# 3DOM-FBK/deep-image-matching

Hardware: AMD Instinct MI355X
Metric: image-pairs/s (SuperPoint+LightGlue, 1024^2, 2048 kpts) (higher is better)
Workload: dtype f32

## Files before the change

### deep-image-matching_amd/csrc/api_ops.hip

```cpp
#include <stdarg.h>
#include <stdio.h>

#include "../../include/dim_hip.h"
#include "sp_kernels.h"

static thread_local char g_err[1024] = "";

void dim_set_error(const char* fmt, ...) {
  va_list ap;
  va_start(ap, fmt);
  vsnprintf(g_err, sizeof(g_err), fmt, ap);
  va_end(ap);
}

#include <vector>
namespace {
unsigned long long g_prof_mask = 0ull;
std::vector<hipEvent_t> g_prof_ev;
size_t g_prof_used = 0;
}

namespace {
constexpr int kMaxDev = 16;
unsigned* g_sat_dev[kMaxDev] = {nullptr};
// ... 85 lines not shown
int dim_follow_stop_flags() { return tuned(18, g_follow_stop); }
static int g_defer_assign = 1;
int dim_defer_assignment() { return tuned(17, g_defer_assign); }
static int g_fuse_ffn_ln = 3;
int dim_fuse_ffn_ln() { return tuned(11, g_fuse_ffn_ln); }
#ifdef DIM_RESEARCH
static int g_gemm_kc = 32;
int dim_gemm_kc() { return g_gemm_kc; }
static int g_conv_wino = 0;
int dim_conv_winograd() { return g_conv_wino; }
static int g_gemm_probe = 0;
int dim_gemm_probe() { return g_gemm_probe; }
static int g_attn_probe = 0;
int dim_attn_probe() { return g_attn_probe; }
#endif
static int g_al_tile_rows = 16;
int dim_aliked_tile_rows() { return tuned(10, g_al_tile_rows); }
static int g_al_fuse_bn = 1;
int dim_aliked_fuse_bn() { return tuned(9, g_al_fuse_bn); }
static int g_presplit = 1;
int dim_presplit_activations() { return tuned(5, g_presplit); }

void dim_prof_begin(int site, hipStream_t s) {
  if (!((g_prof_mask >> site) & 1ull)) return;
  if (g_prof_used + 2 > g_prof_ev.size()) {
    hipEvent_t a, b;
    if (hipEventCreate(&a) != hipSuccess || hipEventCreate(&b) != hipSuccess) return;
    g_prof_ev.push_back(a); g_prof_ev.push_back(b);
  }
  hipEventRecord(g_prof_ev[g_prof_used], s);
// ... 235 lines not shown
  if (key == 0) dim_conv_set_variant(value);
  if (key == 1) g_precision_mode = value;
  if (key == 2) dim_conv_x6_set_variant(value);
  if (key == 3) g_fuse_conv1a = value;
  if (key == 4) g_fold_out_proj = value;
  if (key == 5) g_presplit = value;
  if (key == 6) dim_gemm_x6_set_wide(value);
  if (key == 7) dim_nms_set_big_tiles(value);
  if (key == 8) g_fuse_kv = value;
  if (key == 9) g_al_fuse_bn = value;
  if (key == 10) g_al_tile_rows = value;
  if (key == 11) g_fuse_ffn_ln = value;
  if (key == 16) g_fuse_sp_head = value;
  if (key == 17) g_defer_assign = value;
  if (key == 18) g_follow_stop = value;
#ifdef DIM_RESEARCH
  if (key == 12) g_attn_probe = value;
  if (key == 13) g_gemm_probe = value;
  if (key == 14) g_gemm_kc = value;
  if (key == 15) g_conv_wino = value;
#else
  DIM_REQUIRE(key < 12 || key > 15, "dim_tune_set: key %d selects a research prototype / timing probe that the product library does not contain "
              "(build.build_variant(\"research\", [\"-DDIM_RESEARCH\"]) -> libdim_hip_research.so)", key);
#endif
  DIM_REQUIRE(key >= 0 && key <= 18, "dim_tune_set: unknown key %d", key);
  return 0;
}

int dim_handle_tune_set(void* handle, int key, int value) {
  DimHandleBase* b = (DimHandleBase*)handle;
  DIM_REQUIRE(b != nullptr && b->magic == DIM_HANDLE_MAGIC, "dim_handle_tune_set: not an extractor / matcher handle of this library");
  DIM_REQUIRE(key == 1 || key == 3 || key == 4 || key == 5 || key == 8 || key == 9 || key == 10 || key == 11 || key == 16 || key == 17 || key == 18,
              "dim_handle_tune_set: key %d has no per-handle form (arithmetic 1; fusion 3, 4, 5, 8, 9, 11, 16, 17, 18; ALIKED tile rows 10)", key);
  b->tune.v[key] = value < 0 ? -1 : value;
  return 0;
}

int dim_device_synchronize(void) {
  DIM_HIP(hipDeviceSynchronize());
  return 0;
}

}
```

### deep-image-matching_amd/csrc/conv_x6.hip

```cpp
#include <math.h>
#include <string.h>

#include <type_traits>

#include "dim_kernels.h"

namespace {
constexpr int TW = 32, IW = TW + 2;
constexpr int tile_rows(int mr) { return 4 * mr; }
__host__ __device__ constexpr size_t planes_image_pixels(int h, int w) { return ((size_t)h * w + 1) & ~(size_t)1; }
constexpr int w_slice(int npl) { return npl * 3 * 2 * 64 * 8; }

template <int CIN, int POOL, int PF, bool F1A, int MODE, bool PIN, bool POUT, int MR = 2, bool WDMA = false, bool BN = false>
__global__ __launch_bounds__(256, ((PF == 2 || MR == 4) ? 2 : 3)) void conv3x3_x6_kernel(const float* __restrict__ in, const unsigned short* __restrict__ wx,
                                                            const float* __restrict__ bias, float* __restrict__ out, int H, int W,
                                                            int cout, int relu, int tiles_x, const float* __restrict__ w1a,
                                                            const float* __restrict__ b1a, const float* __restrict__ inv_ch, unsigned* sat,
                                                            unsigned* sat_image) {
  static_assert(!(PIN || POUT) || MODE == 2, "pre-split planes exist for the fp16x3 mode only");
  static_assert(!(PIN && F1A), "the fused conv1a computes its own input");
  using S = SplitMma<MODE>;
  constexpr int NPL = S::NPL, W_SLICE = w_slice(NPL);
  constexpr int TH = tile_rows(MR), IH = TH + 2, NPIX = IH * IW;
  __shared__ u32x4 Ip[NPL * 2 * NPIX];
// ... 266 lines not shown
          const int y = oy + MR * wv + m;
#pragma unroll
          for (int r = 0; r < 16; r += 2) {
            const int x0 = ox + mfma_row(r, half);
            float v0 = acc[m][n][r] * inv_scale + bv, v1 = acc[m][n][r + 1] * inv_scale + bv;
            finish(v0, v1);
            put2((unsigned)(y * W + x0), x0, W, co, cpart, v0, v1);
          }
        }
      }
    }
    if (MODE == 2) sat_report(sat, vmax * (1.0f / OSC));
  };
  if (POOL ? ((ox >> 1) + TW / 2 <= Wo) : (ox + TW <= W)) run_epilogue(std::false_type{});
  else run_epilogue(std::true_type{});
}

__global__ __launch_bounds__(256) void planes_to_f32_kernel(const unsigned short* __restrict__ planes, int C, int hw, float* __restrict__ out, size_t n) {
  const size_t i = (size_t)blockIdx.x * 256 + threadIdx.x;
  if (i >= n) return;
  const size_t gp = i / C, c = i - gp * C, b = gp / hw, pix = gp - b * hw;
  const size_t o = b * planes_image_pixels(hw, 1) * 2 * C + (pix >> 1) * 4 * C + (c >> 4) * 64 + (pix & 1) * 32 + (c & 15);
  const _Float16 hv = __builtin_bit_cast(_Float16, planes[o]), lv = __builtin_bit_cast(_Float16, planes[o + 16]);
  out[i] = ((float)hv + (float)lv) / DIM_F16_ACT_SCALE;
}

unsigned short host_bf16_rne(float x) {
  unsigned u;
  memcpy(&u, &x, 4);
  if ((u & 0x7f800000u) == 0x7f800000u) return (unsigned short)(u >> 16);
// ... 135 lines not shown
    else if (planes_in && planes_out) DIM_CONV6P(CI, P, true, true); \
    else if (planes_in) DIM_CONV6P(CI, P, true, false);        \
    else if (planes_out) DIM_CONV6P(CI, P, false, true);       \
    else DIM_CONV6P(CI, P, false, false);                      \
  }
  if (cin == 64 && pool) DIM_CONV6P_IO(64, 1)
  else if (cin == 64) DIM_CONV6P_IO(64, 0)
  else if (pool) DIM_CONV6P_IO(128, 1)
  else DIM_CONV6P_IO(128, 0)
#undef DIM_CONV6P_IO
#undef DIM_CONV6P
  DIM_LAUNCH_CHECK();
  return 0;
}

int launch_planes_to_f32(const void* planes, int batch, int hw, int channels, float* out, hipStream_t s) {
  const size_t n = (size_t)batch * hw * channels;
  if (n == 0) return 0;
  hipLaunchKernelGGL(planes_to_f32_kernel, dim3((unsigned)((n + 255) / 256)), dim3(256), 0, s, (const unsigned short*)planes, channels, hw, out, n);
  DIM_LAUNCH_CHECK();
  return 0;
}
```

### deep-image-matching_amd/csrc/dim_common.h

```cpp
#pragma once
#include <hip/hip_runtime.h>
#include <stdint.h>

#include <memory>
#include <vector>

typedef float f32x16 __attribute__((ext_vector_type(16)));
typedef float f32x4 __attribute__((ext_vector_type(4)));

typedef __attribute__((ext_vector_type(8))) __bf16 bf16x8;
typedef unsigned int u32x4 __attribute__((ext_vector_type(4)));

#define DIM_WAVE 64

__device__ __forceinline__ f32x16 mfma32(float a, float b, f32x16 c) {
  return __builtin_amdgcn_mfma_f32_32x32x2f32(a, b, c, 0, 0, 0);
}
__device__ __forceinline__ f32x16 mfma_bf16(u32x4 a, u32x4 b, f32x16 c) {
  return __builtin_amdgcn_mfma_f32_32x32x16_bf16(__builtin_bit_cast(bf16x8, a), __builtin_bit_cast(bf16x8, b), c, 0, 0, 0);
}
typedef __attribute__((ext_vector_type(2))) __bf16 bf16x2;
typedef float f32x2 __attribute__((ext_vector_type(2)));
__device__ __forceinline__ unsigned cvt_pk_bf16(float a, float b) {
  f32x2 v = {a, b};
// ... 202 lines not shown
  do {                                                                                \
    hipError_t e__ = hipGetLastError();                                               \
    if (e__ != hipSuccess) {                                                          \
      dim_set_error("kernel launch failed: %s (%s:%d)", hipGetErrorString(e__), __FILE__, __LINE__); \
      return -1;                                                                      \
    }                                                                                 \
  } while (0)
#define DIM_REQUIRE(cond, ...)            \
  do {                                    \
    if (!(cond)) {                        \
      dim_set_error(__VA_ARGS__);         \
      return -2;                          \
    }                                     \
  } while (0)

constexpr int DIM_TUNE_KEYS = 19;
constexpr unsigned DIM_HANDLE_MAGIC = 0x44494d48u;
struct DimTune {
  int v[DIM_TUNE_KEYS];
  DimTune() { for (int i = 0; i < DIM_TUNE_KEYS; ++i) v[i] = -1; }
};
struct DimHandleBase {
  unsigned magic = DIM_HANDLE_MAGIC;
  DimTune tune;
  std::vector<void*> allocs;
  size_t bytes = 0;
};
constexpr size_t DIM_ALLOC_SLACK = 256;
int dim_dev_alloc_bytes(DimHandleBase* b, void** p, size_t bytes);
template <typename T> int dim_dev_alloc(DimHandleBase* b, T** p, size_t count) {
  void* q = nullptr;
// ... 33 lines not shown
```

### deep-image-matching_amd/csrc/dim_kernels.h

```cpp
#pragma once
#include "dim_common.h"

struct SplitWeights {
  const unsigned short* dev = nullptr;
  int mode = 0;
  size_t scale_off = 0;
  int n_pad = 0;
  const float* inv_ch() const { return (const float*)(dev + scale_off); }
};
struct GemmLayerTab { const unsigned short* Bx3; const float* inv_ch; const float* bias; };
struct GemmArgs {
  const float* A0 = nullptr; const float* A1 = nullptr;
  int lda0 = 0, lda1 = 0, ksplit = 0;
  long long strideA0 = 0, strideA1 = 0;
  const int* a_idx = nullptr;
  const float* B = nullptr; int ldb = 0; long long strideB = 0; int bt = 0;
  const unsigned short* Bx3 = nullptr; int n_pad = 0;
  int split_mode = 1; const float* inv_ch = nullptr;
  void set_split(const SplitWeights& w) { Bx3 = w.dev; n_pad = w.n_pad; split_mode = w.mode; inv_ch = w.inv_ch(); }
  unsigned* sat = nullptr;
  const float* bias = nullptr;
  const float* R = nullptr; int ldr = 0; long long strideR = 0;
  float* C = nullptr; int ldc = 0; long long strideC = 0;
  int M = 0, N = 0, K = 0;
// ... 15 lines not shown
int launch_gemm_x6_nt(const GemmArgs& a, int batch, int split_mode, hipStream_t s);
size_t gemm_split_weight_elems(int K, int n_pad, int mode);
void split_weights(const float* w_kn, int K, int N, int n_pad, int mode, unsigned short* out, SplitWeights* sw, int kperm = 0);

int launch_conv3x3(const float* in, const float* w, const float* bias, float* out, int batch, int H, int W,
                   int cin, int cout, int pool, int relu, hipStream_t s);
size_t conv_split_weight_elems(int cin, int cout, int mode);
void prepare_conv_weights_split(const float* w_oihw, int cin, int cout, int mode, unsigned short* out, SplitWeights* sw);
int launch_conv3x3_x6(const float* in, const SplitWeights& wt, const float* bias, float* out, int batch, int H, int W, int cin,
                      int cout, int pool, int relu, hipStream_t s, unsigned* sat = nullptr, int bn = 0);
int launch_conv3x3_x6_fused1a(const float* image, const float* w1a_tap_cout, const float* b1a, const SplitWeights& wt, const float* bias,
                              float* out, int batch, int H, int W, int cout, int pool, int relu, int planes_out, hipStream_t s,
                              unsigned* sat = nullptr, unsigned* sat_image = nullptr, int bn = 0);
int launch_conv3x3_x6_planes(const float* in, const SplitWeights& wt, const float* bias, float* out, int batch, int H, int W, int cin,
                             int cout, int pool, int relu, int planes_in, int planes_out, hipStream_t s, unsigned* sat = nullptr, int bn = 0);
size_t conv_wino_weight_elems(int cin, int cout);
void prepare_conv_weights_wino(const float* w_oihw, int cin, int cout, unsigned short* out, SplitWeights* sw);
int launch_conv3x3_wg_fused1a(const float* image, const float* w1a_tap_cout, const float* b1a, const SplitWeights& wt, const float* bias,
                              float* out, int batch, int H, int W, int cout, int pool, int planes_out, hipStream_t s, unsigned* sat = nullptr,
                              unsigned* sat_image = nullptr);
#ifdef DIM_RESEARCH
int dim_conv_winograd();
#else
static inline int dim_conv_winograd() { return 0; }
#endif
int launch_planes_to_f32(const void* planes, int batch, int hw, int channels, float* out, hipStream_t s);
inline size_t dim_planes_image_pixels(int h, int w) { return ((size_t)h * w + 1) & ~(size_t)1; }
int dim_presplit_activations();
int dim_precision_mode();
int dim_aliked_tile_rows();
// ... 29 lines not shown
```

### deep-image-matching_amd/csrc/sp_api.hip

```cpp
#include <math.h>
#include <stdlib.h>
#include <string.h>

#include <vector>

#include "../../include/dim_hip.h"
#include "sp_kernels.h"

struct dim_sp {
  DimHandleBase base;
  dim_sp_config cfg;
  int max_batch, max_h, max_w, capacity;
  float* w1a; float* wk[12]; float* bias[12];
  SplitWeights wsw[12];
  SplitWeights wsp[3][12];
  float *a1, *b1, *a2, *b2, *a3, *b3, *a4, *x, *pa, *logits, *da, *dd, *smap, *nms, *cand_score;
  int *cand_idx, *rowcount, *rowoff, *ncand;
  unsigned long long* topk_keys;
  int last_h, last_w, last_batch;
  float conv1a_bound;
  bool x_is_planes;
  bool head_fused;
  float* b1_dbg;
  float* x_dbg;
  bool bn;
};

namespace {
const int kCin[12] = {1, 64, 64, 64, 64, 128, 128, 128, 128, 256, 128, 256};
const int kCout[12] = {64, 64, 64, 64, 128, 128, 128, 128, 256, 65, 256, 256};
const int kK[12] = {3, 3, 3, 3, 3, 3, 3, 3, 3, 1, 3, 1};

int sp_create(const dim_sp_weights* w, const std::vector<float>* bn_st, const dim_sp_config* cfg, int max_batch, int max_h, int max_w, int capacity,
              dim_sp** out) {
  DIM_REQUIRE(w && cfg && out, "dim_sp_create: null argument");
  DIM_REQUIRE(max_batch > 0 && max_h >= 8 && max_w >= 8, "dim_sp_create: bad sizes");
  DIM_REQUIRE(cfg->max_keypoints != 0 && cfg->max_keypoints >= -1, "\"max_keypoints\" must be positive or \"-1\"");
  DIM_REQUIRE(capacity > 0 && capacity >= cfg->max_keypoints, "dim_sp_create: capacity %d < max_keypoints %d", capacity, cfg->max_keypoints);
  DIM_REQUIRE(cfg->nms_radius >= 0, "nms_radius must be >= 0");
  std::unique_ptr<dim_sp, void (*)(dim_sp*)> guard(new dim_sp(), dim_sp_destroy);
  dim_sp* const h = guard.get();
  DimHandleBase* const hb = &h->base;
  memset((void*)&h->cfg, 0, sizeof(h->cfg));
  h->cfg = *cfg;
  h->max_batch = max_batch; h->max_h = max_h; h->max_w = max_w; h->capacity = capacity;
  h->last_h = h->last_w = h->last_batch = 0;
  h->b1_dbg = nullptr; h->x_dbg = nullptr; h->head_fused = false;
  h->bn = bn_st != nullptr;
  for (int l = 0; l < 12; ++l) {
    const int ci = kCin[l], co = kCout[l], k = kK[l];
    const int co_pad = (co + 3) & ~3;
    if (!dim_all_finite(w->conv_w[l], (size_t)k * k * ci * co) || !dim_all_finite(w->conv_b[l], (size_t)co)) { dim_set_error("dim_sp_create: non-finite value in the weights of layer %d", l); return -1; }
    std::vector<float> host((size_t)k * k * ci * co_pad, 0.0f);
    for (int o = 0; o < co; ++o)
      for (int i = 0; i < ci; ++i)
        for (int t = 0; t < k * k; ++t) host[((size_t)t * ci + i) * co_pad + o] = w->conv_w[l][((size_t)o * ci + i) * k * k + t];
    if (k == 3 && ci >= 64) {
      for (int mode = 1; mode <= 2; ++mode) {
        std::vector<unsigned short> hx(conv_split_weight_elems(ci, co, mode));
        SplitWeights& sw = h->wsp[mode][l];
        prepare_conv_weights_split(w->conv_w[l], ci, co, mode, hx.data(), &sw);
        DIM_TRY(dim_upload_split(hb, &sw, hx, mode, sw.n_pad));
// ... 26 lines not shown
    if (bn_st) sum = fabsf(bn_st[0][o]) * sum + fabsf(bn_st[0][64 + o]);
    h->conv1a_bound = fmaxf(h->conv1a_bound, sum);
  }
  const size_t B = max_batch, H = max_h, W = max_w;
  const size_t H2 = H / 2, W2 = W / 2, H4 = H2 / 2, W4 = W2 / 2, hh = H4 / 2, ww = W4 / 2;
  h->a1 = nullptr;
  DIM_TRY(dim_dev_alloc(hb, &h->b1, B * dim_planes_image_pixels(H2, W2) * 64));
  DIM_TRY(dim_dev_alloc(hb, &h->a2, B * dim_planes_image_pixels(H2, W2) * 64));
  DIM_TRY(dim_dev_alloc(hb, &h->b2, B * dim_planes_image_pixels(H4, W4) * 64));
  DIM_TRY(dim_dev_alloc(hb, &h->a3, B * dim_planes_image_pixels(H4, W4) * 128));
  DIM_TRY(dim_dev_alloc(hb, &h->b3, B * dim_planes_image_pixels(hh, ww) * 128));
  DIM_TRY(dim_dev_alloc(hb, &h->a4, B * dim_planes_image_pixels(hh, ww) * 128));
  DIM_TRY(dim_dev_alloc(hb, &h->x, B * dim_planes_image_pixels(hh, ww) * 128));
  DIM_TRY(dim_dev_alloc(hb, &h->pa, B * hh * ww * 256));
  DIM_TRY(dim_dev_alloc(hb, &h->logits, B * hh * ww * 65));
  DIM_TRY(dim_dev_alloc(hb, &h->da, B * hh * ww * 256));
  DIM_TRY(dim_dev_alloc(hb, &h->dd, B * hh * ww * 256));
  DIM_TRY(dim_dev_alloc(hb, &h->smap, B * hh * ww * 64));
  DIM_TRY(dim_dev_alloc(hb, &h->nms, B * hh * ww * 64));
  DIM_TRY(dim_dev_alloc(hb, &h->cand_score, B * hh * ww * 64));
  DIM_TRY(dim_dev_alloc(hb, &h->cand_idx, B * hh * ww * 64));
  DIM_TRY(dim_dev_alloc(hb, &h->rowcount, B * hh * 8));
  DIM_TRY(dim_dev_alloc(hb, &h->rowoff, B * hh * 8));
  DIM_TRY(dim_dev_alloc(hb, &h->ncand, B));
  h->topk_keys = nullptr;
  if (topk_scratch_keys(max_batch, cfg->max_keypoints)) DIM_TRY(dim_dev_alloc(hb, &h->topk_keys, topk_scratch_keys(max_batch, cfg->max_keypoints)));
  *out = guard.release();
  return 0;
}
}

extern "C" {
// ... 124 lines not shown
    h->head_fused = pmode == 2 && dim_fuse_sp_head();
    if (h->head_fused) {
      g.set_split(h->wsp[pmode][9]); g.d2s_out = h->smap; g.d2s_h = hh; g.d2s_w = ww;
      DIM_RUN(launch_gemm_x6(g, 1, s));
    } else {
      if (x6) { g.set_split(h->wsp[pmode][9]); DIM_RUN(launch_gemm_x6(g, 1, s)); }
      else DIM_RUN(launch_gemm(g, 1, s));
      DIM_RUN(launch_softmax_d2s(h->logits, h->smap, batch, hh, ww, s));
    }
  }
  DIM_RUN(launch_nms(h->smap, h->nms, batch, H8, W8, h->cfg.nms_radius, s));
  DIM_RUN(launch_select(h->nms, batch, H8, W8, h->cfg.keypoint_threshold, h->cfg.remove_borders, h->rowcount, h->rowoff,
                       h->ncand, h->cand_score, h->cand_idx, s));
  DIM_RUN(launch_topk(h->cand_score, h->cand_idx, h->ncand, batch, H8, W8, h->cfg.max_keypoints, h->capacity, kpts_xy_dev,
                     scores_dev, n_kpts_dev, h->topk_keys, 0, s));
  if (planes) SP_SITE(DIM_PROF_SP_CONVDA, convp(10, h->x, h->da, hh, ww, 128, 256, 0, 1, 0));
  else SP_SITE(DIM_PROF_SP_CONVDA, conv(10, h->x, h->da, hh, ww, 128, 256, 0));
  {
    GemmArgs g;
    g.A0 = h->da; g.lda0 = 256; g.B = h->wk[11]; g.ldb = 256; g.bias = h->bias[11];
    g.C = h->dd; g.ldc = 256; g.M = batch * hh * ww; g.N = 256; g.K = 256;
    if (x6) { g.set_split(h->wsp[pmode][11]); DIM_RUN(launch_gemm_x6(g, 1, s)); }
    else DIM_RUN(launch_gemm(g, 1, s));
  }
  DIM_RUN(launch_sample_desc(h->dd, kpts_xy_dev, n_kpts_dev, desc_dev, batch, hh, ww, h->capacity, h->cfg.fix_sampling, s));
#undef SP_SITE
  h->last_h = hh; h->last_w = ww; h->last_batch = batch;
  return 0;
}

int dim_sp_debug_buffers(dim_sp* h, const float** encoder, const float** logits, const float** score_map,
                         const float** nms_map, const float** dense_desc, int* h8, int* w8) {
  DIM_REQUIRE(h, "dim_sp_debug_buffers: null handle");
  DimTuneScope tune_scope(&h->base);
  if (encoder) {
    *encoder = h->x;
    if (h->x_is_planes) {
      if (!h->x_dbg && dim_dev_alloc(&h->base, &h->x_dbg, (size_t)h->max_batch * (h->max_h / 8) * (h->max_w / 8) * 128) != 0) return -1;
      if (launch_planes_to_f32(h->x, h->last_batch, h->last_h * h->last_w, 128, h->x_dbg, nullptr) != 0) return -1;
      DIM_HIP(hipDeviceSynchronize());
// ... 1 lines not shown
    }
  }
  if (logits) {
    if (h->head_fused && h->last_batch > 0) {
      GemmArgs g;
      g.A0 = h->pa; g.lda0 = 256; g.B = h->wk[9]; g.ldb = 68; g.bias = h->bias[9];
      g.C = h->logits; g.ldc = 65; g.M = h->last_batch * h->last_h * h->last_w; g.N = 65; g.K = 256;
      g.set_split(h->wsp[2][9]);
      if (launch_gemm_x6(g, 1, nullptr) != 0) return -1;
      DIM_HIP(hipDeviceSynchronize());
    }
    *logits = h->logits;
  }
  if (score_map) *score_map = h->smap;
  if (nms_map) *nms_map = h->nms;
  if (dense_desc) *dense_desc = h->dd;
  if (h8) *h8 = h->last_h * 8;
  if (w8) *w8 = h->last_w * 8;
  return 0;
}

int dim_sp_debug_conv1b(dim_sp* h, int batch, int H, int W, const float** out_f32, int* h2, int* w2) {
  DIM_REQUIRE(h && out_f32 && batch >= 1 && batch <= h->max_batch, "dim_sp_debug_conv1b: bad argument");
  DimTuneScope tune_scope(&h->base);
  const int H2 = H / 2, W2 = W / 2;
  if (!h->b1_dbg && dim_dev_alloc(&h->base, &h->b1_dbg, (size_t)h->max_batch * (h->max_h / 2) * (h->max_w / 2) * 64) != 0) return -1;
  const bool planes = h->x_is_planes;
  if (planes) {
    if (launch_planes_to_f32(h->b1, batch, H2 * W2, 64, h->b1_dbg, nullptr) != 0) return -1;
  } else {
    DIM_HIP(hipMemcpy(h->b1_dbg, h->b1, (size_t)batch * H2 * W2 * 64 * sizeof(float), hipMemcpyDeviceToDevice));
  }
  DIM_HIP(hipDeviceSynchronize());
  *out_f32 = h->b1_dbg;
  if (h2) *h2 = H2;
  if (w2) *w2 = W2;
  return 0;
}

int dim_sp_candidate_counts(dim_sp* h, const int32_t** ncand_dev) {
  DIM_REQUIRE(h && ncand_dev, "dim_sp_candidate_counts: null argument");
  *ncand_dev = h->ncand;
  return 0;
}

}
```

### deep-image-matching_amd/csrc/sp_kernels.h

```cpp
#pragma once
#include "dim_kernels.h"

int launch_softmax_d2s(const float* logits, float* smap, int batch, int h, int w, hipStream_t s);
int launch_nms(const float* smap, float* out, int batch, int H8, int W8, int radius, hipStream_t s);
int launch_select(const float* nms, int batch, int H8, int W8, float thr, int border, int* rowcount, int* rowoff,
                  int* ncand, float* cand_score, int* cand_idx, hipStream_t s);
int launch_select_ex(const float* nms, int batch, int H8, int W8, float thr, const float* thr_dev, int border, int* rowcount,
                     int* rowoff, int* ncand, float* cand_score, int* cand_idx, int count_only, hipStream_t s);
size_t topk_scratch_keys(int batch, int k);
int launch_topk(const float* cand_score, const int* cand_idx, const int* ncand, int batch, int H8, int W8, int k,
                int capacity, float* kpts, float* scores, int* n_out, unsigned long long* scratch, int sort_always, hipStream_t s);
int launch_topk_zero_fill(const float* nms, int batch, int H8, int W8, float thr, int border, int k, int capacity, float* kpts, float* scores,
                          int* n_out, hipStream_t s);
int launch_sample_desc(const float* dense, const float* kpts, const int* n_kpts, float* desc, int batch, int h, int w,
                       int capacity, int fix_sampling, hipStream_t s);
```

### deep-image-matching_amd/csrc/sp_post.hip

```cpp
#include <math.h>

#include "sp_kernels.h"

namespace {

constexpr int SD_CPW = 4;
__global__ __launch_bounds__(256) void softmax_d2s_kernel(const float* __restrict__ logits, float* __restrict__ smap,
                                                          int n_cells_total, int h, int w) {
  const int lane = threadIdx.x & 63;
  const int cell0 = (blockIdx.x * 4 + (threadIdx.x >> 6)) * SD_CPW;
  if (cell0 >= n_cells_total) return;
  float v[SD_CPW], dust[SD_CPW];
#pragma unroll
  for (int j = 0; j < SD_CPW; ++j) {
    const float* p = logits + (size_t)min(cell0 + j, n_cells_total - 1) * 65;
    v[j] = p[lane];
    dust[j] = p[64];
  }
  const int W8 = w * 8;
#pragma unroll
  for (int j = 0; j < SD_CPW; ++j) {
    const int cell = cell0 + j;
    if (cell >= n_cells_total) break;
    const float m = fmaxf(wave_max(v[j]), dust[j]);
// ... 491 lines not shown
      all += c;
    }
    const int pos = base + before + __popcll(m & ((1ull << lane) - 1ull));
    if (fill && pos < k) {
      kp[2 * pos] = (float)x;
      kp[2 * pos + 1] = (float)y;
      sc[pos] = 0.0f;
    }
    __syncthreads();
    if (t == 0) sh_base = base + all;
    __syncthreads();
  }
  if (t == 0) n_out[b] = min(sh_base, k);
}

__global__ __launch_bounds__(256) void sample_desc_kernel(const float* __restrict__ dense, const float* __restrict__ kpts,
                                                          const int* __restrict__ n_kpts, float* __restrict__ desc, int h,
                                                          int w, int capacity, int fix_sampling) {
  const int lane = threadIdx.x & 63;
  const int i = blockIdx.x * 4 + (threadIdx.x >> 6), b = blockIdx.y;
  if (i >= n_kpts[b]) return;
  const float kx = kpts[((size_t)b * capacity + i) * 2], ky = kpts[((size_t)b * capacity + i) * 2 + 1];
  float ix, iy;
  if (fix_sampling) {
    float gx = (kx + 0.5f) / ((float)w * 8.0f), gy = (ky + 0.5f) / ((float)h * 8.0f);
    gx = gx * 2.0f - 1.0f; gy = gy * 2.0f - 1.0f;
    ix = ((gx + 1.0f) * (float)w - 1.0f) / 2.0f;
    iy = ((gy + 1.0f) * (float)h - 1.0f) / 2.0f;
  } else {
    float gx = (kx - 4.0f + 0.5f) / ((float)(w * 8) - 4.0f - 0.5f), gy = (ky - 4.0f + 0.5f) / ((float)(h * 8) - 4.0f - 0.5f);
    gx = gx * 2.0f - 1.0f; gy = gy * 2.0f - 1.0f;
    ix = ((gx + 1.0f) / 2.0f) * (float)(w - 1);
    iy = ((gy + 1.0f) / 2.0f) * (float)(h - 1);
  }
  const float fx = floorf(ix), fy = floorf(iy);
  const int x0 = (int)fx, y0 = (int)fy;
  const float wnw = (fx + 1.0f - ix) * (fy + 1.0f - iy), wne = (ix - fx) * (fy + 1.0f - iy);
  const float wsw = (fx + 1.0f - ix) * (iy - fy), wse = (ix - fx) * (iy - fy);
  const float* base = dense + (size_t)b * h * w * 256;
  float acc[4] = {0.f, 0.f, 0.f, 0.f};
  const int cxs[4] = {x0, x0 + 1, x0, x0 + 1};
  const int cys[4] = {y0, y0, y0 + 1, y0 + 1};
  const float wts[4] = {wnw, wne, wsw, wse};
#pragma unroll
  for (int c = 0; c < 4; ++c) {
    const bool in = cxs[c] >= 0 && cxs[c] < w && cys[c] >= 0 && cys[c] < h;
    float4 v = make_float4(0.f, 0.f, 0.f, 0.f);
    if (in) v = *(const float4*)(base + ((size_t)cys[c] * w + cxs[c]) * 256 + lane * 4);
    float ss = wave_sum(v.x * v.x + v.y * v.y + v.z * v.z + v.w * v.w);
    const float den = fmaxf(sqrtf(ss), 1e-12f);
    if (in) {
      acc[0] += (v.x / den) * wts[c]; acc[1] += (v.y / den) * wts[c];
      acc[2] += (v.z / den) * wts[c]; acc[3] += (v.w / den) * wts[c];
    }
  }
  const float ss = wave_sum(acc[0] * acc[0] + acc[1] * acc[1] + acc[2] * acc[2] + acc[3] * acc[3]);
  const float den = fmaxf(sqrtf(ss), 1e-12f);
  *(float4*)(desc + ((size_t)b * capacity + i) * 256 + lane * 4) =
      make_float4(acc[0] / den, acc[1] / den, acc[2] / den, acc[3] / den);
}

}

int launch_softmax_d2s(const float* logits, float* smap, int batch, int h, int w, hipStream_t s) {
  const int n = batch * h * w;
  if (n <= 0) return 0;
  hipLaunchKernelGGL(softmax_d2s_kernel, dim3(cdiv(n, 4 * SD_CPW)), dim3(256), 0, s, logits, smap, n, h, w);
  DIM_LAUNCH_CHECK();
  return 0;
}

static int g_nms_big = 1;
int dim_nms_big_tiles() { return g_nms_big; }
void dim_nms_set_big_tiles(int v) { g_nms_big = v; }
// ... 56 lines not shown
  }
  DIM_LAUNCH_CHECK();
  return 0;
}
int launch_topk_zero_fill(const float* nms, int batch, int H8, int W8, float thr, int border, int k, int capacity, float* kpts, float* scores,
                          int* n_out, hipStream_t s) {
  DIM_REQUIRE(k <= capacity, "topk fill: k %d > capacity %d", k, capacity);
  DIM_REQUIRE((long long)k <= (long long)H8 * W8, "selected index k out of range: top_k %d > %d x %d pixels", k, H8, W8);
  if (batch <= 0) return 0;
  hipLaunchKernelGGL(topk_zero_fill_kernel, dim3(batch), dim3(1024), 0, s, nms, H8, W8, thr, border, k, capacity, kpts, scores, n_out);
  DIM_LAUNCH_CHECK();
  return 0;
}

int launch_sample_desc(const float* dense, const float* kpts, const int* n_kpts, float* desc, int batch, int h, int w,
                       int capacity, int fix_sampling, hipStream_t s) {
  if (batch <= 0 || capacity <= 0) return 0;
  hipLaunchKernelGGL(sample_desc_kernel, dim3(cdiv(capacity, 4), batch), dim3(256), 0, s, dense, kpts, n_kpts, desc, h, w, capacity, fix_sampling);
  DIM_LAUNCH_CHECK();
  return 0;
}
```

### deep-image-matching_amd/superpoint_hip.py

```python
from __future__ import annotations

import ctypes
from typing import Dict, Optional

import torch

from . import capi
from .weights import SP_LAYERS, SPO_BLOCKS, SPO_BN_EPS, validate_superpoint_open_state_dict


class _SpWeights(ctypes.Structure):
    _fields_ = [("conv_w", ctypes.c_void_p * 12), ("conv_b", ctypes.c_void_p * 12)]


class _SpConfig(ctypes.Structure):
    _fields_ = [
        ("nms_radius", ctypes.c_int),
        ("keypoint_threshold", ctypes.c_float),
        ("max_keypoints", ctypes.c_int),
        ("remove_borders", ctypes.c_int),
        ("fix_sampling", ctypes.c_int),
    ]


# ... 19 lines not shown
        c = _SpConfig(int(self.cfg["nms_radius"]), float(self.cfg["keypoint_threshold"]), int(mk),
                      int(self.cfg["remove_borders"]), int(bool(self.cfg["fix_sampling"])))
        self._create(self.lib.dim_sp_create, ctypes.byref(w), ctypes.byref(c), self.max_batch, self.max_hw[0], self.max_hw[1], self.capacity)

    def candidate_counts(self, batch: int) -> torch.Tensor:
        p = ctypes.c_void_p()
        capi.check(self.lib, self.lib.dim_sp_candidate_counts(self._h, ctypes.byref(p)))
        if self.device.type == "cuda":
            torch.cuda.synchronize(self.device)
            out = torch.empty(batch, dtype=torch.int32, device=self.device)
            rc = ctypes.CDLL("libamdhip64.so").hipMemcpy(ctypes.c_void_p(out.data_ptr()), p, ctypes.c_size_t(batch * 4), 3)
            if rc != 0:
                raise capi.DimHipError(f"hipMemcpy failed: {rc}")
            return out.cpu()
        return torch.frombuffer((ctypes.c_int32 * batch).from_address(p.value), dtype=torch.int32).clone()

    @torch.no_grad()
    def extract_batch(self, images: torch.Tensor, out=None):
        assert images.dim() == 3 and images.dtype == torch.float32 and images.is_contiguous()
        B, H, W = images.shape
        dev = images.device
        if out is not None:
            kp, sc, de, n = out
        else:
            kp = torch.empty(B, self.capacity, 2, dtype=torch.float32, device=dev)
            sc = torch.empty(B, self.capacity, dtype=torch.float32, device=dev)
            de = torch.empty(B, self.capacity, 256, dtype=torch.float32, device=dev)
            n = torch.zeros(B, dtype=torch.int32, device=dev)
        with self._ctx():
            capi.check(self.lib, self.lib.dim_sp_extract(self._h, capi.ptr(images), B, H, W, capi.ptr(kp), capi.ptr(sc),
# ... 65 lines not shown
```

### include/dim_hip.h

```cpp
#ifndef DIM_HIP_H
#define DIM_HIP_H

#include <stddef.h>
#include <stdint.h>

#ifdef __cplusplus
extern "C" {
#endif

#define DIM_HIP_ABI_VERSION 2

const char* dim_last_error(void);
int dim_abi_version(void);
int dim_device_synchronize(void);
int dim_tune_set(int key, int value);
int dim_handle_tune_set(void* handle, int key, int value);

enum {
  DIM_PROF_SP_CONV1A = 0, DIM_PROF_SP_CONV1B, DIM_PROF_SP_CONV2A, DIM_PROF_SP_CONV2B, DIM_PROF_SP_CONV3A,
  DIM_PROF_SP_CONV3B, DIM_PROF_SP_CONV4A, DIM_PROF_SP_CONV4B, DIM_PROF_SP_CONVPA, DIM_PROF_SP_CONVPB,
  DIM_PROF_SP_CONVDA, DIM_PROF_SP_CONVDB, DIM_PROF_SP_POST, DIM_PROF_LG_SELF_ATTN, DIM_PROF_LG_CROSS_ATTN,
  DIM_PROF_LG_GEMMS, DIM_PROF_LG_ASSIGN,
  DIM_PROF_AL_CONV_FULL
};
// ... 34 lines not shown
} dim_sp_config;

typedef struct dim_sp dim_sp;

int dim_sp_create(const dim_sp_weights* w, const dim_sp_config* cfg, int max_batch, int max_h, int max_w,
                  int capacity, dim_sp** out);
void dim_sp_destroy(dim_sp* h);

int dim_sp_extract(dim_sp* h, const float* images_dev, int batch, int H, int W, float* kpts_xy_dev, float* scores_dev,
                   float* desc_dev, int32_t* n_kpts_dev, void* stream);

int dim_sp_debug_buffers(dim_sp* h, const float** encoder, const float** logits, const float** score_map,
                         const float** nms_map, const float** dense_desc, int* h8, int* w8);

int dim_sp_debug_conv1b(dim_sp* h, int batch, int H, int W, const float** out_f32, int* h2, int* w2);

int dim_sp_candidate_counts(dim_sp* h, const int32_t** ncand_dev);

typedef struct dim_spo_weights {
  const float* conv_w[12];
  const float* conv_b[12];
  const float* bn_gamma[12];
  const float* bn_beta[12];
  const float* bn_mean[12];
  const float* bn_var[12];
  double bn_eps;
} dim_spo_weights;

int dim_spo_create(const dim_spo_weights* w, const dim_sp_config* cfg, int max_batch, int max_h, int max_w, int capacity, dim_sp** out);

// ... 244 lines not shown
```

Baseline: 616.9.

## Compute descriptor head only at cells touched by keypoint bilinear sampling

```diff
diff --git a/deep-image-matching_amd/csrc/api_ops.hip b/deep-image-matching_amd/csrc/api_ops.hip
--- a/deep-image-matching_amd/csrc/api_ops.hip
+++ b/deep-image-matching_amd/csrc/api_ops.hip
@@ -123,6 +123,12 @@
 static int g_attn_probe = 0;
 int dim_attn_probe() { return g_attn_probe; }
 #endif
+#ifdef DIM_RESEARCH
+int dim_sparse_desc() { return 0; }
+#else
+static int g_sparse_desc = 1;
+int dim_sparse_desc() { return tuned(20, g_sparse_desc); }
+#endif
 static int g_al_tile_rows = 16;
 int dim_aliked_tile_rows() { return tuned(10, g_al_tile_rows); }
 static int g_al_fuse_bn = 1;
@@ -388,6 +394,9 @@
   if (key == 16) g_fuse_sp_head = value;
   if (key == 17) g_defer_assign = value;
   if (key == 18) g_follow_stop = value;
+#ifndef DIM_RESEARCH
+  if (key == 20) g_sparse_desc = value;
+#endif
 #ifdef DIM_RESEARCH
   if (key == 12) g_attn_probe = value;
   if (key == 13) g_gemm_probe = value;
@@ -397,15 +406,15 @@
   DIM_REQUIRE(key < 12 || key > 15, "dim_tune_set: key %d selects a research prototype / timing probe that the product library does not contain "
               "(build.build_variant(\"research\", [\"-DDIM_RESEARCH\"]) -> libdim_hip_research.so)", key);
 #endif
-  DIM_REQUIRE(key >= 0 && key <= 18, "dim_tune_set: unknown key %d", key);
+  DIM_REQUIRE((key >= 0 && key <= 18) || key == 20, "dim_tune_set: unknown key %d", key);
   return 0;
 }
 
 int dim_handle_tune_set(void* handle, int key, int value) {
   DimHandleBase* b = (DimHandleBase*)handle;
   DIM_REQUIRE(b != nullptr && b->magic == DIM_HANDLE_MAGIC, "dim_handle_tune_set: not an extractor / matcher handle of this library");
-  DIM_REQUIRE(key == 1 || key == 3 || key == 4 || key == 5 || key == 8 || key == 9 || key == 10 || key == 11 || key == 16 || key == 17 || key == 18,
-              "dim_handle_tune_set: key %d has no per-handle form (arithmetic 1; fusion 3, 4, 5, 8, 9, 11, 16, 17, 18; ALIKED tile rows 10)", key);
+  DIM_REQUIRE(key == 1 || key == 3 || key == 4 || key == 5 || key == 8 || key == 9 || key == 10 || key == 11 || key == 16 || key == 17 || key == 18 || key == 20,
+              "dim_handle_tune_set: key %d has no per-handle form (arithmetic 1; fusion 3, 4, 5, 8, 9, 11, 16, 17, 18, 20; ALIKED tile rows 10)", key);
   b->tune.v[key] = value < 0 ? -1 : value;
   return 0;
 }
diff --git a/deep-image-matching_amd/csrc/conv_x6.hip b/deep-image-matching_amd/csrc/conv_x6.hip
--- a/deep-image-matching_amd/csrc/conv_x6.hip
+++ b/deep-image-matching_amd/csrc/conv_x6.hip
@@ -304,6 +304,87 @@
   };
   if (POOL ? ((ox >> 1) + TW / 2 <= Wo) : (ox + TW <= W)) run_epilogue(std::false_type{});
   else run_epilogue(std::true_type{});
+}
+
+template <int CIN, int COUT>
+__global__ __launch_bounds__(256, 2) void conv3x3_x6_rows_kernel(const unsigned short* __restrict__ in, const unsigned short* __restrict__ wx,
+                                                                 const float* __restrict__ bias, float* __restrict__ out, int H, int W, int relu,
+                                                                 const float* __restrict__ inv_ch, unsigned* sat, const int* __restrict__ cell_rows,
+                                                                 const int* __restrict__ n_rows, int slots) {
+  using S = SplitMma<2>;
+  constexpr int NPL = 2, W_SLICE = w_slice(NPL), WSL = NPL * 3 * 2 * 64, NCHUNK = CIN / 16, NCB = COUT / 64, NJ = COUT / 32;
+  __shared__ u32x4 Wp[NCB * WSL];
+  const int t = threadIdx.x, lane = t & 63, wv = t >> 6, lx = lane & 31, half = lane >> 5;
+  const int b = blockIdx.y, n = min(n_rows[b], slots), m0 = blockIdx.x * 128;
+  if (m0 >= n) return;
+  const int row = m0 + wv * 32 + lx;
+  const int cell = row < n ? cell_rows[(size_t)b * slots + row] : -1;
+  const int cy = cell / W, cx = cell - cy * W;
+  const unsigned short* pl = in + (size_t)b * planes_image_pixels(H, W) * CIN * 2;
+
+  f32x16 acc[NJ];
+#pragma unroll
+  for (int j = 0; j < NJ; ++j)
+#pragma unroll
+    for (int r = 0; r < 16; ++r) acc[j][r] = 0.0f;
+
+  for (int c = 0; c < NCHUNK; ++c)
+    for (int dy = 0; dy < 3; ++dy) {
+      __syncthreads();
+#pragma unroll
+      for (int cb = 0; cb < NCB; ++cb) {
+        const u32x4* src = (const u32x4*)(wx + ((size_t)(cb * NCHUNK + c) * 3 + dy) * W_SLICE);
+#pragma unroll
+        for (int i = 0; i < WSL / 256; ++i) lds_dma16(src + wv * 64 + 256 * i + lane, &Wp[cb * WSL + wv * 64 + 256 * i]);
+      }
+      u32x4 fa[3][NPL];
+      const int gy = cy + dy - 1;
+#pragma unroll
+      for (int dx = 0; dx < 3; ++dx) {
+        const int gx = cx + dx - 1;
+        const bool ok = cell >= 0 && gy >= 0 && gy < H && gx >= 0 && gx < W;
+        const int pix = ok ? gy * W + gx : 0;
+        const unsigned short* p0 = pl + (size_t)(pix >> 1) * (4 * CIN) + c * 64 + (pix & 1) * 32 + half * 8;
+#pragma unroll
+        for (int p = 0; p < NPL; ++p) {
+          fa[dx][p] = u32x4{0u, 0u, 0u, 0u};
+          if (ok) fa[dx][p] = *(const u32x4*)(p0 + p * 16);
+        }
+      }
+      lds_dma_wait_all();
+      __syncthreads();
+      __builtin_amdgcn_s_setprio(1);
+#pragma unroll
+      for (int dx = 0; dx < 3; ++dx)
+#pragma unroll
+        for (int j = 0; j < NJ; ++j) {
+          u32x4 fb[NPL];
+#pragma unroll
+          for (int p = 0; p < NPL; ++p) fb[p] = Wp[(j >> 1) * WSL + ((p * 3 + dx) * 2 + half) * 64 + (j & 1) * 32 + lx];
+#pragma unroll
+          for (int tm = 0; tm < S::NT; ++tm) acc[j] = S::mma(fa[dx][S::ta(tm)], fb[S::tb(tm)], acc[j]);
+        }
+      __builtin_amdgcn_s_setprio(0);
+    }
+
+  const dim_rsrc rs = buf_rsrc(out + (size_t)b * slots * COUT, (size_t)n * COUT * 4);
+  float vmax = 0.0f;
+#pragma unroll
+  for (int j = 0; j < NJ; ++j) {
+    const int co = j * 32 + lx;
+    const float bv = bias[co], inv_scale = inv_ch[co];
+#pragma unroll
+    for (int r = 0; r < 16; r += 2) {
+      const int r0 = m0 + wv * 32 + mfma_row(r, half);
+      float v0 = acc[j][r] * inv_scale + bv, v1 = acc[j][r + 1] * inv_scale + bv;
+      if (relu) { v0 = fmaxf(v0, 0.0f); v1 = fmaxf(v1, 0.0f); }
+      vmax = sat_track(vmax, r0 < n ? v0 : 0.0f, r0 + 1 < n ? v1 : 0.0f);
+      const unsigned o0 = ((unsigned)r0 * (unsigned)COUT + (unsigned)co) * 4u;
+      buf_store_f32(rs, o0, v0);
+      buf_store_f32(rs, o0 + (unsigned)COUT * 4u, v1);
+    }
+  }
+  sat_report(sat, vmax);
 }
 
 __global__ __launch_bounds__(256) void planes_to_f32_kernel(const unsigned short* __restrict__ planes, int C, int hw, float* __restrict__ out, size_t n) {
@@ -469,6 +550,18 @@
   return 0;
 }
 
+int launch_conv3x3_x6_rows(const float* in_planes, const SplitWeights& wt, const float* bias, float* out_rows, int batch, int H, int W, int cin, int cout,
+                           int relu, const int* cell_rows, const int* n_rows, int slots, hipStream_t s, unsigned* sat) {
+  DIM_REQUIRE(cin == 128 && cout == 256, "conv3x3_x6 rows: cin=%d cout=%d (the 128 -> 256 shape only)", cin, cout);
+  DIM_REQUIRE(wt.dev && wt.mode == 2, "conv3x3_x6 rows: fp16x3 weights required (mode %d)", wt.mode);
+  DIM_REQUIRE(cell_rows && n_rows && slots > 0 && (size_t)slots * cout * 4 < 0x7FFFFFF0ull, "conv3x3_x6 rows: bad row list (%d slots)", slots);
+  if (batch <= 0 || H <= 0 || W <= 0) return 0;
+  hipLaunchKernelGGL(HIP_KERNEL_NAME(conv3x3_x6_rows_kernel<128, 256>), dim3(cdiv(slots, 128), batch), dim3(256), 0, s, (const unsigned short*)in_planes,
+                     wt.dev, bias, out_rows, H, W, relu, wt.inv_ch(), sat, cell_rows, n_rows, slots);
+  DIM_LAUNCH_CHECK();
+  return 0;
+}
+
 int launch_planes_to_f32(const void* planes, int batch, int hw, int channels, float* out, hipStream_t s) {
   const size_t n = (size_t)batch * hw * channels;
   if (n == 0) return 0;
diff --git a/deep-image-matching_amd/csrc/dim_common.h b/deep-image-matching_amd/csrc/dim_common.h
--- a/deep-image-matching_amd/csrc/dim_common.h
+++ b/deep-image-matching_amd/csrc/dim_common.h
@@ -240,7 +240,7 @@
     }                                     \
   } while (0)
 
-constexpr int DIM_TUNE_KEYS = 19;
+constexpr int DIM_TUNE_KEYS = 21;
 constexpr unsigned DIM_HANDLE_MAGIC = 0x44494d48u;
 struct DimTune {
   int v[DIM_TUNE_KEYS];
diff --git a/deep-image-matching_amd/csrc/dim_kernels.h b/deep-image-matching_amd/csrc/dim_kernels.h
--- a/deep-image-matching_amd/csrc/dim_kernels.h
+++ b/deep-image-matching_amd/csrc/dim_kernels.h
@@ -53,6 +53,9 @@
                               unsigned* sat = nullptr, unsigned* sat_image = nullptr, int bn = 0);
 int launch_conv3x3_x6_planes(const float* in, const SplitWeights& wt, const float* bias, float* out, int batch, int H, int W, int cin,
                              int cout, int pool, int relu, int planes_in, int planes_out, hipStream_t s, unsigned* sat = nullptr, int bn = 0);
+int launch_conv3x3_x6_rows(const float* in_planes, const SplitWeights& wt, const float* bias, float* out_rows, int batch, int H, int W, int cin, int cout,
+                           int relu, const int* cell_rows, const int* n_rows, int slots, hipStream_t s, unsigned* sat = nullptr);
+int dim_sparse_desc();
 size_t conv_wino_weight_elems(int cin, int cout);
 void prepare_conv_weights_wino(const float* w_oihw, int cin, int cout, unsigned short* out, SplitWeights* sw);
 int launch_conv3x3_wg_fused1a(const float* image, const float* w1a_tap_cout, const float* b1a, const SplitWeights& wt, const float* bias,
diff --git a/deep-image-matching_amd/csrc/sp_api.hip b/deep-image-matching_amd/csrc/sp_api.hip
--- a/deep-image-matching_amd/csrc/sp_api.hip
+++ b/deep-image-matching_amd/csrc/sp_api.hip
@@ -2,6 +2,7 @@
 #include <stdlib.h>
 #include <string.h>
 
+#include <algorithm>
 #include <vector>
 
 #include "../../include/dim_hip.h"
@@ -24,9 +25,45 @@
   float* b1_dbg;
   float* x_dbg;
   bool bn;
+  float *da_rows, *dd_rows;
+  int *cell_rows, *n_rows, *row_of_cell;
+  int desc_slots;
 };
 
 namespace {
+constexpr double kSparseDescMaxFraction = 0.8;
+
+int sp_alloc_dense_desc(dim_sp* h) {
+  const size_t cells = (size_t)h->max_batch * (h->max_h / 8) * (h->max_w / 8);
+  if (!h->da) DIM_TRY(dim_dev_alloc(&h->base, &h->da, cells * 256));
+  if (!h->dd) DIM_TRY(dim_dev_alloc(&h->base, &h->dd, cells * 256));
+  return 0;
+}
+int sp_alloc_sparse_desc(dim_sp* h) {
+  const size_t hw = (size_t)(h->max_h / 8) * (h->max_w / 8), B = h->max_batch;
+  const size_t slots = std::min((size_t)4 * h->capacity, hw);
+  if (!h->da_rows) DIM_TRY(dim_dev_alloc(&h->base, &h->da_rows, B * slots * 256));
+  if (!h->dd_rows) DIM_TRY(dim_dev_alloc(&h->base, &h->dd_rows, B * slots * 256));
+  if (!h->cell_rows) DIM_TRY(dim_dev_alloc(&h->base, &h->cell_rows, B * slots));
+  if (!h->row_of_cell) DIM_TRY(dim_dev_alloc(&h->base, &h->row_of_cell, B * hw));
+  if (!h->n_rows) DIM_TRY(dim_dev_alloc(&h->base, &h->n_rows, B));
+  return 0;
+}
+int sp_dense_desc(dim_sp* h, int batch, int hh, int ww, int pmode, bool planes, unsigned* sat_head, bool prof, hipStream_t s) {
+  DIM_TRY(sp_alloc_dense_desc(h));
+  if (prof) dim_prof_begin(DIM_PROF_SP_CONVDA, s);
+  if (planes) DIM_RUN(launch_conv3x3_x6_planes(h->x, h->wsp[2][10], h->bias[10], h->da, batch, hh, ww, 128, 256, 0, 1, 1, 0, s, sat_head, 0));
+  else if (pmode != 0) DIM_RUN(launch_conv3x3_x6(h->x, h->wsp[pmode][10], h->bias[10], h->da, batch, hh, ww, 128, 256, 0, 1, s, sat_head, 0));
+  else DIM_RUN(launch_conv3x3(h->x, h->wk[10], h->bias[10], h->da, batch, hh, ww, 128, 256, 0, 1, s));
+  if (prof) dim_prof_end(DIM_PROF_SP_CONVDA, s);
+  GemmArgs g;
+  g.A0 = h->da; g.lda0 = 256; g.B = h->wk[11]; g.ldb = 256; g.bias = h->bias[11];
+  g.C = h->dd; g.ldc = 256; g.M = batch * hh * ww; g.N = 256; g.K = 256;
+  if (pmode != 0) { g.set_split(h->wsp[pmode][11]); DIM_RUN(launch_gemm_x6(g, 1, s)); }
+  else DIM_RUN(launch_gemm(g, 1, s));
+  return 0;
+}
+
 const int kCin[12] = {1, 64, 64, 64, 64, 128, 128, 128, 128, 256, 128, 256};
 const int kCout[12] = {64, 64, 64, 64, 128, 128, 128, 128, 256, 65, 256, 256};
 const int kK[12] = {3, 3, 3, 3, 3, 3, 3, 3, 3, 1, 3, 1};
@@ -46,6 +83,8 @@
   h->max_batch = max_batch; h->max_h = max_h; h->max_w = max_w; h->capacity = capacity;
   h->last_h = h->last_w = h->last_batch = 0;
   h->b1_dbg = nullptr; h->x_dbg = nullptr; h->head_fused = false;
+  h->da = h->dd = nullptr;
+  h->da_rows = h->dd_rows = nullptr; h->cell_rows = h->n_rows = h->row_of_cell = nullptr; h->desc_slots = 0;
   h->bn = bn_st != nullptr;
   for (int l = 0; l < 12; ++l) {
     const int ci = kCin[l], co = kCout[l], k = kK[l];
@@ -102,8 +141,6 @@
   DIM_TRY(dim_dev_alloc(hb, &h->x, B * dim_planes_image_pixels(hh, ww) * 128));
   DIM_TRY(dim_dev_alloc(hb, &h->pa, B * hh * ww * 256));
   DIM_TRY(dim_dev_alloc(hb, &h->logits, B * hh * ww * 65));
-  DIM_TRY(dim_dev_alloc(hb, &h->da, B * hh * ww * 256));
-  DIM_TRY(dim_dev_alloc(hb, &h->dd, B * hh * ww * 256));
   DIM_TRY(dim_dev_alloc(hb, &h->smap, B * hh * ww * 64));
   DIM_TRY(dim_dev_alloc(hb, &h->nms, B * hh * ww * 64));
   DIM_TRY(dim_dev_alloc(hb, &h->cand_score, B * hh * ww * 64));
@@ -258,16 +295,24 @@
                        h->ncand, h->cand_score, h->cand_idx, s));
   DIM_RUN(launch_topk(h->cand_score, h->cand_idx, h->ncand, batch, H8, W8, h->cfg.max_keypoints, h->capacity, kpts_xy_dev,
                      scores_dev, n_kpts_dev, h->topk_keys, 0, s));
-  if (planes) SP_SITE(DIM_PROF_SP_CONVDA, convp(10, h->x, h->da, hh, ww, 128, 256, 0, 1, 0));
-  else SP_SITE(DIM_PROF_SP_CONVDA, conv(10, h->x, h->da, hh, ww, 128, 256, 0));
-  {
+  const int slots = (int)std::min((size_t)4 * h->capacity, (size_t)hh * ww);
+  const int sparse_sel = dim_sparse_desc();
+  const bool sparse = planes && (sparse_sel == 2 || (sparse_sel == 1 && h->cfg.max_keypoints > 0 && (double)slots <= kSparseDescMaxFraction * (double)hh * ww));
+  if (sparse) {
+    DIM_RUN(sp_alloc_sparse_desc(h));
+    DIM_RUN(launch_desc_cell_list(kpts_xy_dev, n_kpts_dev, batch, hh, ww, h->capacity, h->cfg.fix_sampling, slots, h->row_of_cell, h->cell_rows, h->n_rows, s));
+    SP_SITE(DIM_PROF_SP_CONVDA, launch_conv3x3_x6_rows(h->x, h->wsp[2][10], h->bias[10], h->da_rows, batch, hh, ww, 128, 256, 1, h->cell_rows, h->n_rows, slots, s, sat_head));
     GemmArgs g;
-    g.A0 = h->da; g.lda0 = 256; g.B = h->wk[11]; g.ldb = 256; g.bias = h->bias[11];
-    g.C = h->dd; g.ldc = 256; g.M = batch * hh * ww; g.N = 256; g.K = 256;
-    if (x6) { g.set_split(h->wsp[pmode][11]); DIM_RUN(launch_gemm_x6(g, 1, s)); }
-    else DIM_RUN(launch_gemm(g, 1, s));
-  }
-  DIM_RUN(launch_sample_desc(h->dd, kpts_xy_dev, n_kpts_dev, desc_dev, batch, hh, ww, h->capacity, h->cfg.fix_sampling, s));
+    g.A0 = h->da_rows; g.lda0 = 256; g.strideA0 = (long long)slots * 256; g.B = h->wk[11]; g.ldb = 256; g.bias = h->bias[11];
+    g.C = h->dd_rows; g.ldc = 256; g.strideC = (long long)slots * 256; g.M = slots; g.N = 256; g.K = 256; g.rows = h->n_rows;
+    g.set_split(h->wsp[2][11]);
+    DIM_RUN(launch_gemm_x6(g, batch, s));
+    DIM_RUN(launch_sample_desc(h->dd_rows, kpts_xy_dev, n_kpts_dev, desc_dev, batch, hh, ww, h->capacity, h->cfg.fix_sampling, s, h->row_of_cell, slots));
+  } else {
+    DIM_RUN(sp_dense_desc(h, batch, hh, ww, pmode, planes, sat_head, true, s));
+    DIM_RUN(launch_sample_desc(h->dd, kpts_xy_dev, n_kpts_dev, desc_dev, batch, hh, ww, h->capacity, h->cfg.fix_sampling, s));
+  }
+  h->desc_slots = sparse ? slots : 0;
 #undef SP_SITE
   h->last_h = hh; h->last_w = ww; h->last_batch = batch;
   return 0;
@@ -299,7 +344,13 @@
   }
   if (score_map) *score_map = h->smap;
   if (nms_map) *nms_map = h->nms;
-  if (dense_desc) *dense_desc = h->dd;
+  if (dense_desc) {
+    if (h->desc_slots > 0 && h->last_batch > 0) {
+      if (sp_dense_desc(h, h->last_batch, h->last_h, h->last_w, 2, true, nullptr, false, nullptr) != 0) return -1;
+      DIM_HIP(hipDeviceSynchronize());
+    } else if (sp_alloc_dense_desc(h) != 0) return -1;
+    *dense_desc = h->dd;
+  }
   if (h8) *h8 = h->last_h * 8;
   if (w8) *w8 = h->last_w * 8;
   return 0;
@@ -323,6 +374,13 @@
   return 0;
 }
 
+int dim_sp_desc_rows(dim_sp* h, const int32_t** n_rows_dev, int* slots) {
+  DIM_REQUIRE(h && slots, "dim_sp_desc_rows: null argument");
+  *slots = h->desc_slots;
+  if (n_rows_dev) *n_rows_dev = h->desc_slots > 0 ? h->n_rows : nullptr;
+  return 0;
+}
+
 int dim_sp_candidate_counts(dim_sp* h, const int32_t** ncand_dev) {
   DIM_REQUIRE(h && ncand_dev, "dim_sp_candidate_counts: null argument");
   *ncand_dev = h->ncand;
diff --git a/deep-image-matching_amd/csrc/sp_kernels.h b/deep-image-matching_amd/csrc/sp_kernels.h
--- a/deep-image-matching_amd/csrc/sp_kernels.h
+++ b/deep-image-matching_amd/csrc/sp_kernels.h
@@ -13,4 +13,6 @@
 int launch_topk_zero_fill(const float* nms, int batch, int H8, int W8, float thr, int border, int k, int capacity, float* kpts, float* scores,
                           int* n_out, hipStream_t s);
 int launch_sample_desc(const float* dense, const float* kpts, const int* n_kpts, float* desc, int batch, int h, int w,
-                       int capacity, int fix_sampling, hipStream_t s);
+                       int capacity, int fix_sampling, hipStream_t s, const int* row_of_cell = nullptr, int slots = 0);
+int launch_desc_cell_list(const float* kpts, const int* n_kpts, int batch, int h, int w, int capacity, int fix_sampling, int slots, int* row_of_cell,
+                          int* cell_rows, int* n_rows, hipStream_t s);
diff --git a/deep-image-matching_amd/csrc/sp_post.hip b/deep-image-matching_amd/csrc/sp_post.hip
--- a/deep-image-matching_amd/csrc/sp_post.hip
+++ b/deep-image-matching_amd/csrc/sp_post.hip
@@ -529,14 +529,7 @@
   if (t == 0) n_out[b] = min(sh_base, k);
 }
 
-__global__ __launch_bounds__(256) void sample_desc_kernel(const float* __restrict__ dense, const float* __restrict__ kpts,
-                                                          const int* __restrict__ n_kpts, float* __restrict__ desc, int h,
-                                                          int w, int capacity, int fix_sampling) {
-  const int lane = threadIdx.x & 63;
-  const int i = blockIdx.x * 4 + (threadIdx.x >> 6), b = blockIdx.y;
-  if (i >= n_kpts[b]) return;
-  const float kx = kpts[((size_t)b * capacity + i) * 2], ky = kpts[((size_t)b * capacity + i) * 2 + 1];
-  float ix, iy;
+__device__ __forceinline__ void sp_desc_corner(float kx, float ky, int h, int w, int fix_sampling, float& ix, float& iy, int& x0, int& y0) {
   if (fix_sampling) {
     float gx = (kx + 0.5f) / ((float)w * 8.0f), gy = (ky + 0.5f) / ((float)h * 8.0f);
     gx = gx * 2.0f - 1.0f; gy = gy * 2.0f - 1.0f;
@@ -548,11 +541,23 @@
     ix = ((gx + 1.0f) / 2.0f) * (float)(w - 1);
     iy = ((gy + 1.0f) / 2.0f) * (float)(h - 1);
   }
+  x0 = (int)floorf(ix); y0 = (int)floorf(iy);
+}
+
+__global__ __launch_bounds__(256) void sample_desc_kernel(const float* __restrict__ dense, const float* __restrict__ kpts,
+                                                          const int* __restrict__ n_kpts, float* __restrict__ desc, int h,
+                                                          int w, int capacity, int fix_sampling, const int* __restrict__ row_of_cell, int slots) {
+  const int lane = threadIdx.x & 63;
+  const int i = blockIdx.x * 4 + (threadIdx.x >> 6), b = blockIdx.y;
+  if (i >= n_kpts[b]) return;
+  const float kx = kpts[((size_t)b * capacity + i) * 2], ky = kpts[((size_t)b * capacity + i) * 2 + 1];
+  float ix, iy;
+  int x0, y0;
+  sp_desc_corner(kx, ky, h, w, fix_sampling, ix, iy, x0, y0);
   const float fx = floorf(ix), fy = floorf(iy);
-  const int x0 = (int)fx, y0 = (int)fy;
   const float wnw = (fx + 1.0f - ix) * (fy + 1.0f - iy), wne = (ix - fx) * (fy + 1.0f - iy);
   const float wsw = (fx + 1.0f - ix) * (iy - fy), wse = (ix - fx) * (iy - fy);
-  const float* base = dense + (size_t)b * h * w * 256;
+  const float* base = dense + (size_t)b * (row_of_cell ? (size_t)slots : (size_t)h * w) * 256;
   float acc[4] = {0.f, 0.f, 0.f, 0.f};
   const int cxs[4] = {x0, x0 + 1, x0, x0 + 1};
   const int cys[4] = {y0, y0, y0 + 1, y0 + 1};
@@ -561,7 +566,11 @@
   for (int c = 0; c < 4; ++c) {
     const bool in = cxs[c] >= 0 && cxs[c] < w && cys[c] >= 0 && cys[c] < h;
     float4 v = make_float4(0.f, 0.f, 0.f, 0.f);
-    if (in) v = *(const float4*)(base + ((size_t)cys[c] * w + cxs[c]) * 256 + lane * 4);
+    if (in) {
+      size_t row = (size_t)cys[c] * w + cxs[c];
+      if (row_of_cell) row = (size_t)row_of_cell[(size_t)b * h * w + row];
+      v = *(const float4*)(base + row * 256 + lane * 4);
+    }
     float ss = wave_sum(v.x * v.x + v.y * v.y + v.z * v.z + v.w * v.w);
     const float den = fmaxf(sqrtf(ss), 1e-12f);
     if (in) {
@@ -573,6 +582,48 @@
   const float den = fmaxf(sqrtf(ss), 1e-12f);
   *(float4*)(desc + ((size_t)b * capacity + i) * 256 + lane * 4) =
       make_float4(acc[0] / den, acc[1] / den, acc[2] / den, acc[3] / den);
+}
+
+__global__ __launch_bounds__(256) void mark_desc_cells_kernel(const float* __restrict__ kpts, const int* __restrict__ n_kpts, int h, int w, int capacity,
+                                                              int fix_sampling, int* __restrict__ row_of_cell) {
+  const int i = blockIdx.x * 256 + threadIdx.x, b = blockIdx.y;
+  if (i >= min(n_kpts[b], capacity)) return;
+  const float kx = kpts[((size_t)b * capacity + i) * 2], ky = kpts[((size_t)b * capacity + i) * 2 + 1];
+  float ix, iy;
+  int x0, y0;
+  sp_desc_corner(kx, ky, h, w, fix_sampling, ix, iy, x0, y0);
+  int* m = row_of_cell + (size_t)b * h * w;
+#pragma unroll
+  for (int c = 0; c < 4; ++c) {
+    const int cx = x0 + (c & 1), cy = y0 + (c >> 1);
+    if (cx >= 0 && cx < w && cy >= 0 && cy < h) m[cy * w + cx] = 0;
+  }
+}
+
+__global__ __launch_bounds__(1024) void compact_desc_cells_kernel(int* __restrict__ row_of_cell, int* __restrict__ cell_rows, int* __restrict__ n_rows,
+                                                                  int hw, int slots) {
+  __shared__ int part[1024];
+  const int t = threadIdx.x, b = blockIdx.x;
+  int* m = row_of_cell + (size_t)b * hw;
+  const int per = (hw + 1023) / 1024;
+  const int c0 = min(t * per, hw), c1 = min(c0 + per, hw);
+  int sum = 0;
+  for (int c = c0; c < c1; ++c) sum += m[c] >= 0 ? 1 : 0;
+  part[t] = sum;
+  __syncthreads();
+  for (int off = 1; off < 1024; off <<= 1) {
+    int v = (t >= off) ? part[t - off] : 0;
+    __syncthreads();
+    part[t] += v;
+    __syncthreads();
+  }
+  int run = part[t] - sum;
+  for (int c = c0; c < c1; ++c)
+    if (m[c] >= 0) {
+      if (run < slots) { cell_rows[(size_t)b * slots + run] = c; m[c] = run; }
+      ++run;
+    }
+  if (t == 1023) n_rows[b] = min(part[1023], slots);
 }
 
 }
@@ -659,9 +710,19 @@
 }
 
 int launch_sample_desc(const float* dense, const float* kpts, const int* n_kpts, float* desc, int batch, int h, int w,
-                       int capacity, int fix_sampling, hipStream_t s) {
+                       int capacity, int fix_sampling, hipStream_t s, const int* row_of_cell, int slots) {
   if (batch <= 0 || capacity <= 0) return 0;
-  hipLaunchKernelGGL(sample_desc_kernel, dim3(cdiv(capacity, 4), batch), dim3(256), 0, s, dense, kpts, n_kpts, desc, h, w, capacity, fix_sampling);
+  hipLaunchKernelGGL(sample_desc_kernel, dim3(cdiv(capacity, 4), batch), dim3(256), 0, s, dense, kpts, n_kpts, desc, h, w, capacity, fix_sampling, row_of_cell, slots);
   DIM_LAUNCH_CHECK();
   return 0;
 }
+
+int launch_desc_cell_list(const float* kpts, const int* n_kpts, int batch, int h, int w, int capacity, int fix_sampling, int slots, int* row_of_cell,
+                          int* cell_rows, int* n_rows, hipStream_t s) {
+  if (batch <= 0 || capacity <= 0 || h <= 0 || w <= 0) return 0;
+  DIM_HIP(hipMemsetAsync(row_of_cell, 0xFF, (size_t)batch * h * w * sizeof(int), s));
+  hipLaunchKernelGGL(mark_desc_cells_kernel, dim3(cdiv(capacity, 256), batch), dim3(256), 0, s, kpts, n_kpts, h, w, capacity, fix_sampling, row_of_cell);
+  hipLaunchKernelGGL(compact_desc_cells_kernel, dim3(batch), dim3(1024), 0, s, row_of_cell, cell_rows, n_rows, h * w, slots);
+  DIM_LAUNCH_CHECK();
+  return 0;
+}
diff --git a/deep-image-matching_amd/superpoint_hip.py b/deep-image-matching_amd/superpoint_hip.py
--- a/deep-image-matching_amd/superpoint_hip.py
+++ b/deep-image-matching_amd/superpoint_hip.py
@@ -57,6 +57,20 @@
                 raise capi.DimHipError(f"hipMemcpy failed: {rc}")
             return out.cpu()
         return torch.frombuffer((ctypes.c_int32 * batch).from_address(p.value), dtype=torch.int32).clone()
+
+    def desc_rows(self, batch: int):
+        p, slots = ctypes.c_void_p(), ctypes.c_int()
+        capi.check(self.lib, self.lib.dim_sp_desc_rows(self._h, ctypes.byref(p), ctypes.byref(slots)))
+        if slots.value == 0:
+            return None
+        if self.device.type == "cuda":
+            torch.cuda.synchronize(self.device)
+            out = torch.empty(batch, dtype=torch.int32, device=self.device)
+            rc = ctypes.CDLL("libamdhip64.so").hipMemcpy(ctypes.c_void_p(out.data_ptr()), p, ctypes.c_size_t(batch * 4), 3)
+            if rc != 0:
+                raise capi.DimHipError(f"hipMemcpy failed: {rc}")
+            return slots.value, out.cpu()
+        return slots.value, torch.frombuffer((ctypes.c_int32 * batch).from_address(p.value), dtype=torch.int32).clone()
 
     @torch.no_grad()
     def extract_batch(self, images: torch.Tensor, out=None):
diff --git a/include/dim_hip.h b/include/dim_hip.h
--- a/include/dim_hip.h
+++ b/include/dim_hip.h
@@ -72,6 +72,8 @@
                          const float** nms_map, const float** dense_desc, int* h8, int* w8);
 
 int dim_sp_debug_conv1b(dim_sp* h, int batch, int H, int W, const float** out_f32, int* h2, int* w2);
+
+int dim_sp_desc_rows(dim_sp* h, const int32_t** n_rows_dev, int* slots);
 
 int dim_sp_candidate_counts(dim_sp* h, const int32_t** ncand_dev);
 
```

New measurement: 626.0 (median of 6 runs). +1.5%, better.
